# andreadiiorio/SpMV_openMP_CUDA

Measured on AMD Instinct MI355X. Metric: spmv_gflops, higher is better.
Workload: dtype f64

## Files before the change

### include/spmvHip.h

```cpp
#ifndef SPMV_HIP_H
#define SPMV_HIP_H

#include "spmv_types.h"

#ifdef __cplusplus
extern "C" {
#endif

int spmvHipInit(int dev, size_t sizeofSpmat, size_t sizeofConfig);
int spmvHipFinalize(void);
int spmvHipDeviceCount(void);
int spmvHipSetStream(void* stream);
int spmvHipSetSync(int sync);
double spmvHipLastKernelSeconds(void);
int spmvHipLastLaunch(spmvDim3* grid, spmvDim3* block);
int spmvHipDeviceSynchronize(void);

int spmvHipVecAlloc(double** dVec, size_t n);
int spmvHipVecFree(double* dVec);
int spmvHipVecUp(double* dVec, const double* hVec, size_t n);
int spmvHipVecDown(double* hVec, const double* dVec, size_t n);
int spmvHipVecFill(double* dVec, size_t n, uint64_t pattern);

int spmvHipMalloc(void** dPtr, size_t bytes);
// ... 349 lines not shown
    int      taper, ntStore;
    unsigned chunk;
    double   buildMs;
    size_t   bytes;
    double   allocMs;
    size_t   tempBytes;
    int      deterministic;
} spmvTilesInfo;
int spmvHipTilesInfo(spmat* dMat, spmvTilesInfo* info);
int spmvHipTilesBinRow(spmat* dMat, unsigned bin, ulong* firstRow);
int hipSpMVTilesExpand(spmat* dMat, double* dX);
int hipSpMVTilesReduce(spmat* dMat, unsigned binBegin, unsigned binEnd, double* dY, int nExtra, double* const* dExtra);
int hipSpMVTilesReducePush(spmat* dMat, double* dY, int nExtra, double* const* dExtra);
int spmvHipTilesPushJoin(void);
int spmvHipTilesPushFailed(spmat* dMat);

int spmvHipSynthFillCSR(ulong M, ulong N, ulong rowOffset, const void* dIRP, int irpBytes,
                        uint32_t* dJA, double* dAS, uint64_t seedStruct, uint64_t seedVal,
                        ulong band);

#ifdef __cplusplus
}
#endif
#endif
```

### spmv_openmp_cuda_amd/api.py

```python
import contextlib
import ctypes as C
import math
import os

import numpy as np

from .ctypes_defs import CONFIG, POISON_NAN, SPMAT_TAG_ELL_TRANSPOSED, spmat, spmvDim3

_HERE = os.path.dirname(os.path.abspath(__file__))
LIB_PATH = os.environ.get("SPMV_LIB") or os.path.join(_HERE, "lib", "libspmvhip.so")
HOSTLIB_PATH = os.path.join(_HERE, "lib", "libspmvhost.so")


class SpmvHipError(RuntimeError):
    pass


def _load(path):
    if not os.path.exists(path):
        raise SpmvHipError(
            f"{path} is missing: build it with `make lib host` (or __graft_entry__.build()). "
            "This package has no CPU fallback.")
    return C.CDLL(path, mode=C.RTLD_GLOBAL)

# ... 50 lines not shown
    "spmvHipDropCache": ([], _i),
    "spmvHipEventCreate": ([C.POINTER(_vp)], _i), "spmvHipEventDestroy": ([_vp], _i),
    "spmvHipEventRecord": ([_vp], _i), "spmvHipEventElapsedMs": ([_vp, _vp, C.POINTER(C.c_float)], _i),
    "spmvHipPartitionRows": ([_vp, C.c_ulong, _i, _vp], _i),
    "spmvHipRowBlockCSR": ([C.POINTER(spmat), C.c_ulong, C.c_ulong], C.POINTER(spmat)),
    "spmvHipSynthFillCSR": ([C.c_ulong, C.c_ulong, C.c_ulong, _vp, _i, _vp, _vp, _u64, _u64, C.c_ulong], _i),
    "spmvHipCompactRows": ([_vp, _vp, _vp, _i, C.c_ulong], _i),
    "spmvHipWindowCreate": ([_sz, C.POINTER(_vp), _vp], _i), "spmvHipWindowFree": ([_vp], _i),
    "spmvHipWindowOpen": ([_vp, _i, C.POINTER(_vp)], _i), "spmvHipWindowClose": ([_vp], _i),
    "spmvHipPeerPush": ([_vp, _sz, _sz, _i, _vp], _i), "spmvHipPeerPushJoin": ([], _i),
    "spmvHipTilesShape": ([C.POINTER(spmat), C.POINTER(C.c_uint), C.POINTER(C.c_uint)], _i),
    "hipSpMVTilesExpand": ([C.POINTER(spmat), _vp], _i),
    "hipSpMVTilesReduce": ([C.POINTER(spmat), C.c_uint, C.c_uint, _vp, _i, _vp], _i),
    "hipSpMVTilesReducePush": ([C.POINTER(spmat), _vp, _i, _vp], _i), "spmvHipTilesPushFailed": ([C.POINTER(spmat)], _i),
    "spmvHipTilesPushJoin": ([], _i),
    "spmvHipBuildTilesOpt": ([C.POINTER(spmat), _vp], _i), "spmvHipTilesInfo": ([C.POINTER(spmat), _vp], _i),
    "spmvHipTilesBinRow": ([C.POINTER(spmat), C.c_uint, C.POINTER(C.c_ulong)], _i),
    "spmvHipUpdateValues": ([C.POINTER(spmat), _vp, _i], _i), "spmvHipValuesChanged": ([C.POINTER(spmat)], _i),
    "spmvHipLastUpdateInfo": ([C.POINTER(spmat), _vp], _i), "spmvHipShardUpdateValues": ([_vp, _vp], _i),
    "hipSpMMRowsCSR": ([C.POINTER(spmat), C.c_uint, _vp, _sz, _i, _vp, _sz, _i], _i),
    "spmvHipCsrTranspose": ([C.POINTER(spmat), C.POINTER(spmat)], _i),
    "spmvHipTransposeRefresh": ([C.POINTER(spmat), C.POINTER(spmat)], _i),
    "spmvHipTriAnalyse": ([C.POINTER(spmat), _i], _i),
    "hipSpTRSVCSR": ([C.POINTER(spmat), _i, _i, _vp, _vp], _i),
    "spmvHipTriInfo": ([C.POINTER(spmat), _i, _vp], _i),
    "hipSpTRSMCSR": ([C.POINTER(spmat), _i, _i, C.c_uint, _vp, _sz, _i, _vp, _sz, _i], _i),
    "hipSpILU0CSR": ([C.POINTER(spmat)], _i),
    "spmvHipIlu0Info": ([C.POINTER(spmat), _vp], _i),
    "spmvHipDot": ([_sz, _vp, _vp, _vp], _i),
    "hipSpCGCSR": ([C.POINTER(spmat), C.POINTER(spmat), _vp, _vp, _vp, _vp], _i),
# ... 1122 lines not shown
    fn = SPMV_LAUNCHERS[launcher]
    _check(fn(C.byref(dmat.handle), dx.ptr, cfg if cfg is not None else CONFIG(), dy.ptr), launcher)


def build_tiles(dmat: DeviceMatrix, rowsPerBin=0, taper=False, ntStore=-1, chunk=0, deterministic=False):
    o = spmvTilesOpts(int(rowsPerBin), 1 if taper else 0, int(ntStore), int(chunk), 1 if deterministic else 0)
    _check(lib.spmvHipBuildTilesOpt(C.byref(dmat.handle), C.byref(o)), "spmvHipBuildTilesOpt")


def tiles_info(dmat: DeviceMatrix) -> spmvTilesInfo:
    info = spmvTilesInfo()
    _check(lib.spmvHipTilesInfo(C.byref(dmat.handle), C.byref(info)), "spmvHipTilesInfo")
    return info


def build_stripes(dmat: DeviceMatrix, rowsPerBin=0, grid=0, spread=-1, wide=-1, deterministic=False):
    o = spmvStripesOpts(int(rowsPerBin), int(grid), int(spread), int(wide), int(deterministic))
    _check(lib.spmvHipBuildStripesOpt(C.byref(dmat.handle), C.byref(o)), "spmvHipBuildStripesOpt")


def stripes_info(dmat: DeviceMatrix) -> spmvStripesInfo:
    info = spmvStripesInfo()
    _check(lib.spmvHipStripesInfo(C.byref(dmat.handle), C.byref(info)), "spmvHipStripesInfo")
    return info


def dot(u, v):
    with _Operands("dot", u, host_calls=False) as ops:
        n = ops.vector("u", u)
        ops.vector("v", v, n)
# ... 43 lines not shown
```

### spmv_openmp_cuda_amd/csrc/hip/device_mat.hpp

```cpp
#pragma once
#include <hip/hip_runtime.h>
#include <atomic>
#include <cstdint>
#include <cstdio>
#include <type_traits>
#include <vector>

#include "spmvHip.h"

namespace spmvhip {

constexpr int      WAVE            = 64;
constexpr int      WG_THREADS      = 256;
constexpr int      STREAM_NNZ      = 2048;
constexpr uint64_t IRP32_LIMIT     = (1ull << 32) - 65536;

enum class Kind : int { CSR = 0, ELL_ROWMAJOR = 1, ELL_COLMAJOR = 2 };
enum class Origin : int { UPLOADED, ADOPTED, ELL_OF_CSR, TRANSPOSE, PERMUTATION, PRODUCT, HIERARCHY, SUM, FILTER, ASSEMBLED };

struct TileFormat;
struct SellFormat;
struct StripeFormat;
struct SpgemmPlan;
struct AddPlan;
// ... 81 lines not shown
int  enqueueStripes(const StripeFormat* f, const double* x, double* y, hipStream_t stream, int mode, dim3* grid = nullptr, dim3* block = nullptr);
size_t stripesBytes(const DevMat* d);
void stripesInfo(const StripeFormat* f, spmvStripesInfo* out);

int  buildTiles(DevMat* d, const spmvTilesOpts* opts = nullptr);
void tilesInfo(const TileFormat* t, spmvTilesInfo* out);
void freeTiles(TileFormat* t);
void peerFinalize();
void freeTilesWorkspace();
int  enqueueTiles(const DevMat* d, const TileFormat* t, const double* x, double* y, hipStream_t stream);
int  enqueueTilesExpand(const DevMat* d, const TileFormat* t, const double* x, hipStream_t stream);
int  enqueueTilesReduce(const DevMat* d, const TileFormat* t, uint32_t binBegin, uint32_t binEnd, double* y, int nExtra, double* const* extra,
                        hipStream_t stream);
int  enqueueTilesReducePush(const DevMat* d, TileFormat* t, double* y, int nExtra, double* const* extra, hipStream_t stream, hipStream_t side,
                            hipEvent_t evFork, hipEvent_t evJoin);
int  tilesPushFailed(const TileFormat* t);
void tilesShape(const TileFormat* t, uint32_t* bins, uint32_t* rowsPerBin);
uint32_t tilesPhase2Threads(const TileFormat* t);
uint64_t tilesBinRow(const DevMat* d, const TileFormat* t, uint32_t bin);
hipStream_t libraryStream();
size_t tilesBytes(const DevMat* d);

int  tilesRefreshValues(DevMat* d, TileFormat* t, hipStream_t stream, double* mapMs, int* mapsBuilt);
int  stripesRefreshValues(DevMat* d, StripeFormat* f, hipStream_t stream, double* mapMs, int* mapsBuilt);
bool stripesHasValues(const StripeFormat* f);
spmvStripesOpts stripesOptions(const StripeFormat* f);
void stripesSetUnit(StripeFormat* f, bool unit, double value);
int  sellRefreshValues(DevMat* d, hipStream_t stream);
int  transposeCsr(const DevMat* a, DevMat* t, hipStream_t stream);
void enqueueSortedBounds(uint64_t nnz, uint64_t N, const uint32_t* keys, uint32_t* ptr, hipStream_t stream);
// ... 121 lines not shown
```

### spmv_openmp_cuda_amd/csrc/hip/launch.hip

```cpp
#include <hip/hip_runtime.h>

#include "lib.hpp"

using namespace spmvhip;

namespace {

unsigned blockThreads(const CONFIG& cfg, unsigned dflt, unsigned maxThreads) {
    unsigned t = cfg.blockSize.x * std::max(1u, cfg.blockSize.y) * std::max(1u, cfg.blockSize.z);
    if (cfg.blockSize.x == 0) return dflt;
    if (t % WAVE != 0 || t > maxThreads) {
        ERR("CONFIG.blockSize %ux%ux%u is not a multiple of the 64-lane wavefront (or exceeds %u): using %u",
            cfg.blockSize.x, cfg.blockSize.y, cfg.blockSize.z, maxThreads, dflt);
        return dflt;
    }
    return t;
}

template <bool SEQ>
void launchStream2(hipStream_t stream, DevMat* d, double* x, double* y) {
    withIrp(d, [&](auto irp) {
        const auto kernel = d->unit ? csr_stream2_kernel<IrpT<decltype(irp)>, SEQ, true> : csr_stream2_kernel<IrpT<decltype(irp)>, SEQ, false>;
        hipLaunchKernelGGL(kernel, grid2d(d->nBlk2, WG_THREADS), dim3(WG_THREADS), 0, stream,
                           d->nBlk2, d->nLong2, d->blkInfo, d->blkBase, irp, d->JA, d->AS, d->unitValue, x, y);
// ... 293 lines not shown
}

int hipSpMVTilesReduce(spmat* dMat, unsigned binBegin, unsigned binEnd, double* dY, int nExtra, double* const* dExtra) {
    const Ctx cx = libraryCtx();
    const auto [d, t] = tilesReady(dMat, "hipSpMVTilesReduce");
    if (!t) return EXIT_FAILURE;
    uint32_t b = 0, r = 0;
    tilesShape(t, &b, &r);
    if (binBegin > binEnd || binEnd > b || nExtra < 0 || nExtra > SPMV_MAX_PEERS || (nExtra && !dExtra) || !dY) {
        ERR("hipSpMVTilesReduce: bins [%u,%u) of %u, %d extra destinations: invalid", binBegin, binEnd, b, nExtra);
        return EXIT_FAILURE;
    }
    Launch L(cx, dim3(binEnd - binBegin ? binEnd - binBegin : 1), dim3(1024));
    if (enqueueTilesReduce(d, t, binBegin, binEnd, dY, nExtra, dExtra, cx.stream)) { ERR("hipSpMVTilesReduce: launch failed"); return EXIT_FAILURE; }
    return L.finish("hipSpMVTilesReduce");
}

int hipSpMVTilesReducePush(spmat* dMat, double* dY, int nExtra, double* const* dExtra) {
    const Ctx cx = libraryCtx();
    const auto [d, t] = tilesReady(dMat, "hipSpMVTilesReducePush");
    if (!t) return EXIT_FAILURE;
    if (nExtra < 1 || nExtra > SPMV_MAX_PEERS || !dExtra || !dY) { ERR("hipSpMVTilesReducePush: %d destinations: invalid", nExtra); return EXIT_FAILURE; }
    if (!g_pushSide) {
        int lo = 0, hi = 0;
        HIP_TRY(hipDeviceGetStreamPriorityRange(&lo, &hi));
        HIP_TRY(hipStreamCreateWithPriority(&g_pushSide, hipStreamNonBlocking, hi));
        HIP_TRY(hipEventCreateWithFlags(&g_pushFork, hipEventDisableTiming));
        HIP_TRY(hipEventCreateWithFlags(&g_pushJoin, hipEventDisableTiming));
    }
    uint32_t b = 0, r = 0;
// ... 37 lines not shown
```

### spmv_openmp_cuda_amd/csrc/hip/tiles.hip

```cpp
#include <hip/hip_runtime.h>
#include <cstring>
#include <cmath>
#include <chrono>
#include <algorithm>
#include <vector>

#include "spmvHip.h"
#include "kernels.hpp"
#include "device_prims.hpp"

namespace spmvhip {

constexpr uint32_t PB_CBITS   = 14;
constexpr uint32_t PB_C       = 1u << PB_CBITS;
static_assert(PB_C % 1024 == 0 && PB_C * 8 <= 160 * 1024 && PB_C <= 65536, "slice width");
constexpr uint32_t PB_R_MAX   = 20000;
constexpr uint32_t PB_CUS_DEFAULT = 256;
constexpr uint32_t PB_CHUNK   = 1u << 17;
constexpr int      PB_THREADS = 1024;
constexpr uint32_t PD_WAVES   = 4;
constexpr int      PD_THREADS = PD_WAVES * 64;
constexpr size_t   PB_RESIDENT_BYTES = 288ull << 20;

struct BinMap {
// ... 12 lines not shown
struct TileFormat {
    uint32_t S = 0, B = 0, R = 0;
    BinMap    bins;
    uint64_t nnz = 0;
    void*     slab = nullptr;
    double*   val = nullptr;
    uint16_t* lcol = nullptr;
    uint16_t* lrow = nullptr;
    bool      det = false;
    uint32_t* pidx = nullptr;
    size_t    tempBytes = 0;
    uint2*    tl = nullptr;
    uint32_t  nList = 0;
    uint32_t* binPos = nullptr;
    uint32_t* waveTile = nullptr;
    uint3*    work = nullptr;
    uint32_t  nWork = 0;
    uint32_t* runs = nullptr;
    uint32_t  grid1 = 0;
    bool      ntStore = true;
    uint32_t* ready = nullptr;
    uint32_t* pushFail = nullptr;
    uint32_t  epoch = 0;
    uint32_t  cus = PB_CUS_DEFAULT;
    size_t    bytes = 0;
    spmvTilesOpts opts{0, 0, -1, 0, 0};
    uint32_t apiBins() const { return det ? (B + PD_WAVES - 1) / PD_WAVES : B; }
    uint32_t apiRows() const { return det ? PD_WAVES * bins.c : R; }
    BinMap   apiMap() const { if (!det) return bins; BinMap m; m.c = PD_WAVES * bins.c; return m; }
    uint32_t  chunk = 0;
    double    buildMs = 0;
    double    allocMs = 0;
    uint32_t* vmap = nullptr;
};

struct TileDst { double* p[SPMV_MAX_PEERS]; uint32_t n; };
struct TileSignal { uint32_t* ready; uint32_t epoch; };

namespace {

__device__ __forceinline__ uint64_t lin_block() { return (uint64_t)blockIdx.y * gridDim.x + blockIdx.x; }

struct PbPay { uint32_t vlo, vhi, row; };
static_assert(sizeof(PbPay) == 12 && alignof(PbPay) == 4, "payload layout");
__host__ __device__ __forceinline__ PbPay pb_pack(double v, uint32_t row) {
    uint64_t b;
    memcpy(&b, &v, 8);
    return PbPay{(uint32_t)b, (uint32_t)(b >> 32), row};
}
__host__ __device__ __forceinline__ double pb_value(const PbPay& e) {
    const uint64_t b = ((uint64_t)e.vhi << 32) | e.vlo;
    double v;
    memcpy(&v, &b, 8);
    return v;
}

// ... 58 lines not shown
    uint32_t S, uint32_t B, BinMap bm, const uint32_t* __restrict__ tileStart, const uint32_t* __restrict__ bmStart,
    double* __restrict__ val, uint16_t* __restrict__ lcol, uint16_t* __restrict__ lrow, uint32_t* __restrict__ pidx) {
    const uint64_t p = lin_block() * 256 + threadIdx.x;
    if (p >= nnz) return;
    const PbPay e = spay[p];
    const uint32_t key = skeys[p];
    const uint32_t bin = bm.binOf(e.row), slice = key >> PB_CBITS;
    val[p] = pb_value(e);
    lcol[p] = (uint16_t)(key & (PB_C - 1));
    const uint32_t within = (uint32_t)p - tileStart[(uint64_t)slice * B + bin];
    const uint32_t at = bmStart[(uint64_t)bin * S + slice] + within;
    lrow[at] = (uint16_t)(e.row - bm.row0(bin));
    if (pidx) pidx[at] = (uint32_t)p;
}

__global__ __launch_bounds__(256) void pb_fill_kernel(uint32_t* p, uint64_t n, uint32_t v) {
    const uint64_t i = lin_block() * 256 + threadIdx.x;
    if (i < n) p[i] = v;
}

__global__ __launch_bounds__(256) void pb_invert_kernel(uint64_t n, const uint32_t* __restrict__ perm, uint32_t* __restrict__ inv) {
    const uint64_t p = lin_block() * 256 + threadIdx.x;
    if (p < n) inv[perm[p]] = (uint32_t)p;
}

typedef double   dbl2 __attribute__((ext_vector_type(2)));
typedef uint16_t ush2 __attribute__((ext_vector_type(2)));

constexpr int      P1_DEPTH = 8;
constexpr uint32_t P1_STEP  = 2 * PB_THREADS;
// ... 39 lines not shown

template <uint32_t I0, uint32_t I1>
__device__ __forceinline__ void p1_load_x(double (&xv)[I1 - I0], uint32_t slice, const double* __restrict__ x, uint64_t N) {
    const double* xb = x + (uint64_t)slice * PB_C;
    const uint32_t nIn = (uint32_t)min(N - (uint64_t)slice * PB_C, (uint64_t)PB_C);
#pragma unroll
    for (uint32_t i = I0; i < I1; ++i)
        xv[i - I0] = xb[min(threadIdx.x + i * PB_THREADS, nIn - 1)];
}
template <uint32_t I0, uint32_t I1>
__device__ __forceinline__ void p1_fill_x(double* xs, const double (&xv)[I1 - I0]) {
#pragma unroll
    for (uint32_t i = I0; i < I1; ++i) xs[threadIdx.x + i * PB_THREADS] = xv[i - I0];
}

template <bool NT, bool UNIT>
__global__ __launch_bounds__(PB_THREADS) void pb_expand_kernel(
    const uint32_t* __restrict__ runs, const uint3* __restrict__ work, const double* __restrict__ val,
    const uint16_t* __restrict__ lcol, const double* __restrict__ x, uint64_t N, double* __restrict__ prod, double unitValue) {
    extern __shared__ double xs[];
    constexpr uint32_t BATCH = P1_DEPTH * P1_STEP;
    uint32_t item = runs[blockIdx.x];
    const uint32_t itemEnd = runs[blockIdx.x + 1];
    if (item >= itemEnd) return;
    const uint32_t lane2 = 2 * threadIdx.x;

    uint3 w = work[item];
    P1Range r = p1_range(w);
    P1Regs cur, nxt;
    double xv[P1_XPRE];
    p1_load_x<0, P1_XPRE>(xv, w.x, x, N);
    p1_load<UNIT>(cur, r.vb + lane2, r.ve, val, lcol, unitValue);
    bool restage = true;

    for (;;) {
        if (restage) {
            __syncthreads();
            double xr[P1_XALL - P1_XPRE];
// ... 14 lines not shown
        uint32_t pb = r.vb;
        do {
            last = pb + 2 * BATCH >= r.ve;
            const uint32_t p = pb + lane2;
            p1_load<UNIT>(nxt, p + BATCH, r.ve, val, lcol, unitValue);
            p1_store<NT>(cur, p, r.ve, xs, prod);
            if (last && restage) p1_load_x<0, P1_XPRE>(xv, wn.x, x, N);
            const bool hand = last && more;
            p1_load<UNIT>(cur, hand ? rn.vb + lane2 : p + 2 * BATCH, hand ? rn.ve : r.ve, val, lcol, unitValue);
            p1_store<NT>(nxt, p + BATCH, r.ve, xs, prod);
            pb += 2 * BATCH;
        } while (!last);
        if (!more) break;
        w = wn; r = rn; ++item;
    }
}

constexpr int      P2_DEPTH = 8;
constexpr uint32_t P2_WAVES = PB_THREADS / 64;
constexpr uint16_t P2_NONE  = 0xFFFF;
constexpr uint32_t P2_RUNS_FLAG = 0x80000000u;
constexpr uint32_t TL_PAD   = 4;

__host__ __device__ __forceinline__ uint32_t p2_sub(uint32_t len) { return ((len + P2_WAVES - 1) / P2_WAVES + 63u) & ~63u; }

struct P2Regs { double pv[P2_DEPTH]; uint16_t rv[P2_DEPTH]; };
struct P2Cursor { uint32_t k, delta; uint2 n1, n2; };

__device__ __forceinline__ void p2_fetch(P2Regs& r, P2Cursor& c, uint32_t vbase, uint32_t we, uint32_t lane,
                                         const uint2* __restrict__ tl, const double* __restrict__ prod,
// ... 55 lines not shown
            for (uint32_t k = threadIdx.x; k < R; k += THREADS)
                if (r0 + k < M) dst[r0 + k] = yb[k];
        }
    }
    if (MODE == 2) {
        asm volatile("s_waitcnt vmcnt(0)" ::: "memory");
        __syncthreads();
        if (threadIdx.x == 0) {
            __builtin_amdgcn_fence(__ATOMIC_RELEASE, "agent");
            asm volatile("s_waitcnt vmcnt(0)" ::: "memory");
            __hip_atomic_store(sig.ready + bin, sig.epoch, __ATOMIC_RELAXED, __HIP_MEMORY_SCOPE_AGENT);
        }
    }
}

template <int MODE>
__global__ __launch_bounds__(PB_THREADS) void pb_reduce_kernel(
    BinMap bm, uint32_t binBegin, uint32_t binEnd, uint64_t M, const uint32_t* __restrict__ binPos, const uint32_t* __restrict__ waveTile,
    const uint2* __restrict__ tl, const double* __restrict__ prod, const uint16_t* __restrict__ lrow,
    double* __restrict__ y, TileDst extra, TileSignal sig) {
    extern __shared__ double yb[];
    const uint64_t bin = binBegin + lin_block();
    if (bin >= binEnd) return;
    const uint32_t wave = (uint32_t)__builtin_amdgcn_readfirstlane((int)(threadIdx.x / 64)), lane = threadIdx.x % 64;
    const uint32_t v0 = binPos[bin], v1 = binPos[bin + 1];
    const uint32_t sub = p2_sub(v1 - v0);
    const uint32_t wb = v0 + wave * sub, we = min(v1, wb + sub);
    P2Cursor c;
    P2Regs a, b;
    bool runs = false;
    const bool busy = wave * sub < v1 - v0;
    if (busy) {
        const uint32_t wt = waveTile[bin * P2_WAVES + wave];
        runs = (wt & P2_RUNS_FLAG) != 0;
        c.k = wt & ~P2_RUNS_FLAG;
        c.delta = tl[c.k].y;
        c.n1 = tl[c.k + 1];
        c.n2 = tl[c.k + 2];
// ... 15 lines not shown
                    if (b.rv[u] != P2_NONE) atomicAdd(&yb[b.rv[u]], b.pv[u]);
            }
        } else {
            for (uint32_t v = wb; v < we; v += 2 * P2_DEPTH * 64) {
                p2_fetch(b, c, v + P2_DEPTH * 64, we, lane, tl, prod, lrow);
#pragma unroll
                for (int u = 0; u < P2_DEPTH; ++u) p2_add_runs(yb, a.rv[u], a.pv[u], lane);
                p2_fetch(a, c, v + 2 * P2_DEPTH * 64, we, lane, tl, prod, lrow);
#pragma unroll
                for (int u = 0; u < P2_DEPTH; ++u) p2_add_runs(yb, b.rv[u], b.pv[u], lane);
            }
        }
    }
    __syncthreads();
    p2_finish<MODE, PB_THREADS>(yb, R, bm.row0((uint32_t)bin), M, y, extra, sig, (uint32_t)bin);
}

constexpr int PD_DEPTH = 8;
struct PdStream { uint32_t idx[PD_DEPTH]; uint16_t row[PD_DEPTH]; uint32_t first; };
struct PdGather { double p[PD_DEPTH]; };

__device__ __forceinline__ void pd_stream(PdStream& s, uint32_t vb, uint32_t we, uint32_t lane, const uint32_t* __restrict__ pidx,
                                          const uint16_t* __restrict__ lrow) {
    s.first = vb;
#pragma unroll
    for (int u = 0; u < PD_DEPTH; ++u) {
        const uint32_t v = vb + 64u * u + lane, vc = min(v, we - 1u);
        s.idx[u] = __builtin_nontemporal_load(pidx + vc);
        const uint16_t r = __builtin_nontemporal_load(lrow + vc);
        s.row[u] = v < we ? r : P2_NONE;
// ... 1 lines not shown
}
__device__ __forceinline__ void pd_gather(PdGather& g, const PdStream& s, const double* __restrict__ prod) {
#pragma unroll
    for (int u = 0; u < PD_DEPTH; ++u) g.p[u] = prod[s.idx[u]];
}
__device__ __forceinline__ void pd_add(double* yw, const PdStream& s, const PdGather& g) {
#pragma unroll
    for (int u = 0; u < PD_DEPTH; ++u)
        if (s.row[u] != P2_NONE) atomicAdd(&yw[s.row[u]], g.p[u]);
}

template <int MODE>
__global__ __launch_bounds__(PD_THREADS) void pb_reduce_det_kernel(
    BinMap bm, uint32_t nSub, uint32_t binBegin, uint32_t binEnd, uint64_t M, const uint32_t* __restrict__ binPos,
    const uint32_t* __restrict__ pidx, const double* __restrict__ prod, const uint16_t* __restrict__ lrow,
    double* __restrict__ y, TileDst extra, TileSignal sig) {
    extern __shared__ double yb[];
    const uint64_t bin = binBegin + lin_block();
    if (bin >= binEnd) return;
    const uint32_t wave = (uint32_t)__builtin_amdgcn_readfirstlane((int)(threadIdx.x / 64)), lane = threadIdx.x % 64;
    const uint32_t sb = (uint32_t)bin * PD_WAVES + wave;
    const uint32_t Rs = bm.c;
    double* yw = yb + wave * Rs;
    uint32_t wb = 0, we = 0;
    if (sb < nSub) { wb = binPos[sb]; we = binPos[sb + 1]; }
    const bool busy = we > wb;
    constexpr uint32_t BATCH = PD_DEPTH * 64;
    PdStream a, b, c, d;
    PdGather g0, g1;
    if (busy) {
        pd_stream(a, wb, we, lane, pidx, lrow);
        pd_stream(b, wb + BATCH, we, lane, pidx, lrow);
        pd_stream(c, wb + 2 * BATCH, we, lane, pidx, lrow);
    }
// ... 182 lines not shown
            if (g_prod[d].lastUse) (void)hipEventDestroy(g_prod[d].lastUse);
            g_prod[d] = ProdWorkspace{};
        }
    (void)hipSetDevice(keep);
}

uint64_t tilesBinRow(const DevMat* d, const TileFormat* t, uint32_t bin) {
    if (!t) return 0;
    return bin >= t->apiBins() ? d->M : std::min<uint64_t>(d->M, t->apiMap().row0(bin));
}

void freeTiles(TileFormat* t) {
    if (!t) return;
    (void)devFree(t->slab); (void)devFree(t->tl); (void)devFree(t->pidx); (void)devFree(t->vmap);
    (void)devFree(t->binPos); (void)devFree(t->waveTile); (void)devFree(t->work); (void)devFree(t->runs); (void)devFree(t->ready);
    delete t;
}

static int buildFailed(const char* what) { (void)hipGetLastError(); fprintf(stderr, "libspmvhip: tiles: %s failed\n", what); return EXIT_FAILURE; }

static int checkTilesBuild(const DevMat* d, const spmvTilesOpts& o) {
    if (d->kind != Kind::CSR) return EXIT_FAILURE;
    if (o.deterministic && o.taper) { fprintf(stderr, "libspmvhip: tiles: the deterministic form has no tapered bins\n"); return EXIT_FAILURE; }
    if (o.rowsPerBin != 0 && (o.rowsPerBin < 64 || o.rowsPerBin > PB_R_MAX)) {
        fprintf(stderr, "libspmvhip: tiles: rowsPerBin = %u is not 0 (automatic) or 64..%u\n", o.rowsPerBin, PB_R_MAX);
        return EXIT_FAILURE;
    }
    if (o.chunk != 0 && (o.chunk < 4096 || o.chunk > (1u << 24))) {
        fprintf(stderr, "libspmvhip: tiles: chunk = %u is not 0 (automatic) or 4096..2^24\n", o.chunk);
        return EXIT_FAILURE;
// ... 118 lines not shown
        TempBuf dupCount;
        if (dupCount.alloc((size_t)t->B * P2_WAVES * 4)) return buildFailed("run-count workspace");
        HIP_TRY(hipMemsetAsync(dupCount.p, 0, (size_t)t->B * P2_WAVES * 4, nullptr));
        hipLaunchKernelGGL(pb_dupcount_kernel, grid2d((nnz + 255) / 256, 256), dim3(256), 0, nullptr, t->B, nnz, t->binPos, t->lrow,
                           dupCount.as<uint32_t>());
        hipLaunchKernelGGL(pb_wavetile_kernel, grid2d(((uint64_t)t->B * P2_WAVES + 255) / 256, 256), dim3(256), 0, nullptr, t->B,
                           t->binPos, binTile.as<uint32_t>(), t->tl, dupCount.as<uint32_t>(), t->waveTile);
        HIP_TRY(hipGetLastError());
        HIP_TRY(hipDeviceSynchronize());
    }
    HIP_TRY(hipGetLastError());
    HIP_TRY(hipDeviceSynchronize());
    return EXIT_SUCCESS;
}

static uint32_t phase1Chunk(const std::vector<uint32_t>& sliceStart, uint64_t nnz, uint32_t PB_CUS) {
    uint32_t chunk = PB_CHUNK;
    uint64_t nonEmpty = 0;
    for (size_t s = 0; s + 1 < sliceStart.size(); ++s) nonEmpty += sliceStart[s + 1] > sliceStart[s];
    const double avgLen = nonEmpty ? (double)nnz / (double)nonEmpty : 1.0;
    double bestCost = 1e300;
    const uint32_t pLo = (uint32_t)std::max(1.0, std::ceil(avgLen / 100000.0));
    const uint32_t pHi = (uint32_t)std::max((double)pLo, std::ceil(avgLen / 50000.0));
    for (uint32_t p = pLo; p <= std::min<uint32_t>(pHi, 1024); ++p) {
        const double rounds = (double)nonEmpty * p / PB_CUS;
        const double waste = (std::ceil(rounds) - rounds) / rounds;
        const double cost = 0.35 * waste + 0.1 * p * (PB_C * 8.0) / (avgLen * 18.0);
        if (cost < bestCost) { bestCost = cost; chunk = (uint32_t)std::min(16777216.0, std::ceil(avgLen / p * 1.02) + 64); }
    }
    return chunk;
// ... 28 lines not shown
            if (c > b) { plan.work.push_back(make_uint3(it.x, b, c)); b = c; }
            plan.runs[g] = (uint32_t)plan.work.size();
        }
        plan.work.push_back(make_uint3(it.x, b, it.z));
    }
    for (; g <= grid; ++g) plan.runs[g] = (uint32_t)plan.work.size();
    return plan;
}

static int setTilesKernelAttributes() {
    const struct { const void* kernel; int ldsBytes; } attrs[] = {
        {(const void*)pb_expand_kernel<true, false>, PB_C * 8}, {(const void*)pb_expand_kernel<false, false>, PB_C * 8},
        {(const void*)pb_expand_kernel<true, true>, PB_C * 8},  {(const void*)pb_expand_kernel<false, true>, PB_C * 8},
        {(const void*)pb_reduce_kernel<0>, PB_R_MAX * 8},       {(const void*)pb_reduce_kernel<1>, PB_R_MAX * 8},
        {(const void*)pb_reduce_kernel<2>, PB_R_MAX * 8},       {(const void*)pb_reduce_det_kernel<0>, PB_R_MAX * 8},
        {(const void*)pb_reduce_det_kernel<1>, PB_R_MAX * 8},   {(const void*)pb_reduce_det_kernel<2>, PB_R_MAX * 8}};
    for (const auto& a : attrs) HIP_TRY(hipFuncSetAttribute(a.kernel, hipFuncAttributeMaxDynamicSharedMemorySize, a.ldsBytes));
    return EXIT_SUCCESS;
}

int buildTiles(DevMat* d, const spmvTilesOpts* opts) {
    const spmvTilesOpts o = opts ? *opts : spmvTilesOpts{0, 0, -1, 0, 0};
    TileFormat*& slot = d->tiles[o.deterministic != 0];
    if (slot && !opts) return EXIT_SUCCESS;
    if (checkTilesBuild(d, o)) return EXIT_FAILURE;
    if (slot) { freeTiles(slot); slot = nullptr; }
    const uint64_t nnz = d->NZ;
    TileFormat* t = new TileFormat;
    struct Guard { TileFormat*& t; ~Guard() { if (t) freeTiles(t); } } guard{t};
    {
        int dev = 0, cus = 0;
// ... 2 lines not shown
    }
    hipEvent_t ev0 = nullptr, ev1 = nullptr;
    HIP_TRY(hipEventCreate(&ev0));
    HIP_TRY(hipEventCreate(&ev1));
    struct EvGuard { hipEvent_t a, b; ~EvGuard() { (void)hipEventDestroy(a); (void)hipEventDestroy(b); } } evGuard{ev0, ev1};
    HIP_TRY(hipEventRecord(ev0, nullptr));
    const TileGeometry g = planTileBins(d->M, t->cus, o);
    t->opts = o;
    t->S = (uint32_t)((d->N + PB_C - 1) / PB_C);
    t->bins = g.bins; t->R = g.R; t->B = g.B;
    t->det = o.deterministic != 0;
    t->nnz = nnz;
    if ((uint64_t)t->S * t->B >= (1ull << 32) - 2) { fprintf(stderr, "libspmvhip: tiles: too many tiles\n"); return EXIT_FAILURE; }

    TileBuildTemps tmp;
    if (sortIntoSlices(d, t, tmp) || placeTiles(t, tmp)) return EXIT_FAILURE;

    std::vector<uint32_t> sliceStart(t->S + 1);
    HIP_TRY(hipMemcpy2D(sliceStart.data(), 4, tmp.tileStart.as<uint32_t>(), (size_t)t->B * 4, 4, t->S + 1, hipMemcpyDeviceToHost));
    t->chunk = o.chunk ? o.chunk : phase1Chunk(sliceStart, nnz, t->cus);
    const Phase1Plan plan = planPhase1Work(sliceStart, t->chunk, t->cus);
    t->nWork = (uint32_t)plan.work.size();
    t->grid1 = plan.runs.empty() ? 0 : (uint32_t)plan.runs.size() - 1;
    HIP_TRY(devMalloc(&t->work, std::max<size_t>(plan.work.size(), 1) * sizeof(uint3)));
    HIP_TRY(hipMemcpy(t->work, plan.work.data(), plan.work.size() * sizeof(uint3), hipMemcpyHostToDevice));
    HIP_TRY(devMalloc(&t->runs, std::max<size_t>(plan.runs.size(), 1) * sizeof(uint32_t)));
    HIP_TRY(hipMemcpy(t->runs, plan.runs.data(), plan.runs.size() * sizeof(uint32_t), hipMemcpyHostToDevice));
    HIP_TRY(hipDeviceSynchronize());

    if (setTilesKernelAttributes()) return EXIT_FAILURE;
    t->ntStore = o.ntStore >= 0 ? o.ntStore != 0 : nnz * 8 > PB_RESIDENT_BYTES;
// ... 46 lines not shown
void tilesInfo(const TileFormat* t, spmvTilesInfo* out) {
    memset(out, 0, sizeof *out);
    if (!t) return;
    out->nBins = t->apiBins(); out->rowsPerBin = t->apiRows(); out->nSlices = t->S; out->taper = t->bins.n1 != 0; out->ntStore = t->ntStore;
    out->chunk = t->chunk; out->buildMs = t->buildMs; out->bytes = t->bytes; out->allocMs = t->allocMs;
    out->tempBytes = t->tempBytes; out->deterministic = t->det ? 1 : 0;
}

uint32_t tilesPhase2Threads(const TileFormat* t) { return t && t->det ? (uint32_t)PD_THREADS : (uint32_t)PB_THREADS; }

void tilesShape(const TileFormat* t, uint32_t* bins, uint32_t* rowsPerBin) {
    *bins = t ? t->apiBins() : 0;
    *rowsPerBin = t ? t->apiRows() : 0;
}

int enqueueTilesExpand(const DevMat* d, const TileFormat* t, const double* x, hipStream_t stream) {
    if (!t) return EXIT_FAILURE;
    double* prod = prodWorkspace(t->nnz, true);
    if (!prod || prodHandover(stream)) return EXIT_FAILURE;
    if (t->nWork) {
#define PB_EXPAND(NT, UNIT) hipLaunchKernelGGL((pb_expand_kernel<NT, UNIT>), dim3(t->grid1), dim3(PB_THREADS), PB_C * 8, stream, t->runs, t->work, \
                                              t->val, t->lcol, x, d->N, prod, d->unitValue)
        if (d->unit) { if (t->ntStore) PB_EXPAND(true, true); else PB_EXPAND(false, true); }
        else         { if (t->ntStore) PB_EXPAND(true, false); else PB_EXPAND(false, false); }
#undef PB_EXPAND
    }
    return hipGetLastError() == hipSuccess ? EXIT_SUCCESS : EXIT_FAILURE;
}

int enqueueTilesReduce(const DevMat* d, const TileFormat* t, uint32_t binBegin, uint32_t binEnd, double* y, int nExtra, double* const* extra,
                       hipStream_t stream) {
    if (!t || binBegin > binEnd || binEnd > t->apiBins() || nExtra < 0 || nExtra > SPMV_MAX_PEERS) return EXIT_FAILURE;
    if (binBegin == binEnd) return EXIT_SUCCESS;
    const dim3 grid = grid2d((uint64_t)((binEnd - binBegin + 7) / 8) * 8, PB_THREADS);
    const double* prod = prodWorkspace(t->nnz, false);
    if (!prod || prodHandover(stream)) return EXIT_FAILURE;
    TileDst dst{};
    dst.n = (uint32_t)nExtra;
    for (int i = 0; i < nExtra; ++i) dst.p[i] = extra[i];
    const TileSignal none{nullptr, 0};
    if (t->det) {
        const size_t lds = (size_t)8 * t->apiRows();
        if (nExtra)
            hipLaunchKernelGGL(pb_reduce_det_kernel<1>, grid, dim3(PD_THREADS), lds, stream, t->bins, t->B, binBegin, binEnd, d->M, t->binPos,
                               t->pidx, prod, t->lrow, y, dst, none);
        else
            hipLaunchKernelGGL(pb_reduce_det_kernel<0>, grid, dim3(PD_THREADS), lds, stream, t->bins, t->B, binBegin, binEnd, d->M, t->binPos,
                               t->pidx, prod, t->lrow, y, dst, none);
        const bool launched = hipGetLastError() == hipSuccess;
        prodMark(stream);
        return launched ? EXIT_SUCCESS : EXIT_FAILURE;
    }
    if (nExtra)
        hipLaunchKernelGGL(pb_reduce_kernel<1>, grid, dim3(PB_THREADS), (size_t)8 * t->R, stream,
                           t->bins, binBegin, binEnd, d->M, t->binPos, t->waveTile, t->tl, prod, t->lrow, y, dst, none);
    else
        hipLaunchKernelGGL(pb_reduce_kernel<0>, grid, dim3(PB_THREADS), (size_t)8 * t->R, stream,
                           t->bins, binBegin, binEnd, d->M, t->binPos, t->waveTile, t->tl, prod, t->lrow, y, dst, none);
    const bool launched = hipGetLastError() == hipSuccess;
    prodMark(stream);
    return launched ? EXIT_SUCCESS : EXIT_FAILURE;
}

int enqueueTilesReducePush(const DevMat* d, TileFormat* t, double* y, int nExtra, double* const* extra, hipStream_t stream, hipStream_t side,
                           hipEvent_t evFork, hipEvent_t evJoin) {
    if (!t || nExtra < 1 || nExtra > SPMV_MAX_PEERS) return EXIT_FAILURE;
    const double* prod = prodWorkspace(t->nnz, true);
    if (!prod || prodHandover(stream)) return EXIT_FAILURE;
    const uint32_t nb = t->apiBins();
    if (!t->ready) {
        if (!hipOk(devMalloc(&t->ready, ((size_t)nb + 1) * 4), "hipMalloc of the bins' ready flags")) return EXIT_FAILURE;
        if (hipMemset(t->ready, 0, ((size_t)nb + 1) * 4) != hipSuccess) return EXIT_FAILURE;
        t->pushFail = t->ready + nb;
    }
    const uint32_t epoch = ++t->epoch ? t->epoch : ++t->epoch;
    TileDst dst{};
    dst.n = (uint32_t)nExtra;
    for (int i = 0; i < nExtra; ++i) dst.p[i] = extra[i];
    const TileSignal sig{t->ready, epoch};
    if (hipEventRecord(evFork, stream) != hipSuccess || hipStreamWaitEvent(side, evFork, 0) != hipSuccess) return EXIT_FAILURE;
    hipLaunchKernelGGL(pb_push_kernel, dim3(std::min<uint32_t>(PUSH_WGS, nb)), dim3(PUSH_THREADS), 0, side, t->apiMap(), nb, d->M, t->ready,
                       epoch, y, dst, t->pushFail);
    if (t->det)
        hipLaunchKernelGGL(pb_reduce_det_kernel<2>, grid2d((uint64_t)((nb + 7) / 8) * 8, PB_THREADS), dim3(PD_THREADS), (size_t)8 * t->apiRows(), stream,
                           t->bins, t->B, 0u, nb, d->M, t->binPos, t->pidx, prod, t->lrow, y, TileDst{}, sig);
    else
        hipLaunchKernelGGL(pb_reduce_kernel<2>, grid2d((uint64_t)((t->B + 7) / 8) * 8, PB_THREADS), dim3(PB_THREADS), (size_t)8 * t->R, stream,
                           t->bins, 0u, t->B, d->M, t->binPos, t->waveTile, t->tl, prod, t->lrow, y, TileDst{}, sig);
    const bool launched = hipGetLastError() == hipSuccess;
    prodMark(stream);
    if (hipEventRecord(evJoin, side) != hipSuccess) return EXIT_FAILURE;
    return launched ? EXIT_SUCCESS : EXIT_FAILURE;
}

int tilesPushFailed(const TileFormat* t) {
    if (!t || !t->pushFail) return 0;
    uint32_t f = 0;
    if (hipMemcpy(&f, t->pushFail, 4, hipMemcpyDeviceToHost) != hipSuccess) return 1;
    return f != 0;
}

int enqueueTiles(const DevMat* d, const TileFormat* t, const double* x, double* y, hipStream_t stream) {
    if (!t) return EXIT_FAILURE;
    if (enqueueTilesExpand(d, t, x, stream)) return EXIT_FAILURE;
    return enqueueTilesReduce(d, t, 0, t->apiBins(), y, 0, nullptr, stream);
}

}
```

Baseline: 402.3.

## Schedule reduce bins heaviest-first via sorted bin order and add stamp probes

At build time the bins are sorted by descending nonzero count, and the reduce kernels index bins through this order when they cover the whole range. The longest bins therefore start first, which is meant to cut tail imbalance in the reduce phase. The change also adds wall-clock stamp instrumentation entry points for per-workgroup timing. The cost is one extra indirection load per workgroup and a sort step during build.

After: 394.4. -2.0%, worse.

```diff
diff --git a/include/spmvHip.h b/include/spmvHip.h
--- a/include/spmvHip.h
+++ b/include/spmvHip.h
@@ -387,6 +387,8 @@
 int hipSpMVTilesReducePush(spmat* dMat, double* dY, int nExtra, double* const* dExtra);
 int spmvHipTilesPushJoin(void);
 int spmvHipTilesPushFailed(spmat* dMat);
+int spmvHipTilesFinishSpread(spmat* dMat, double* dX, double* dY, double out[6]);
+int spmvHipTilesFinishStamps(spmat* dMat, int phase, unsigned cap, double* entryUs, double* exitUs, unsigned* count);
 
 int spmvHipSynthFillCSR(ulong M, ulong N, ulong rowOffset, const void* dIRP, int irpBytes,
                         uint32_t* dJA, double* dAS, uint64_t seedStruct, uint64_t seedVal,
diff --git a/spmv_openmp_cuda_amd/api.py b/spmv_openmp_cuda_amd/api.py
--- a/spmv_openmp_cuda_amd/api.py
+++ b/spmv_openmp_cuda_amd/api.py
@@ -88,6 +88,8 @@
     "hipSpMVTilesReduce": ([C.POINTER(spmat), C.c_uint, C.c_uint, _vp, _i, _vp], _i),
     "hipSpMVTilesReducePush": ([C.POINTER(spmat), _vp, _i, _vp], _i), "spmvHipTilesPushFailed": ([C.POINTER(spmat)], _i),
     "spmvHipTilesPushJoin": ([], _i),
+    "spmvHipTilesFinishSpread": ([C.POINTER(spmat), _vp, _vp, C.POINTER(C.c_double)], _i),
+    "spmvHipTilesFinishStamps": ([C.POINTER(spmat), _i, C.c_uint, _vp, _vp, C.POINTER(C.c_uint)], _i),
     "spmvHipBuildTilesOpt": ([C.POINTER(spmat), _vp], _i), "spmvHipTilesInfo": ([C.POINTER(spmat), _vp], _i),
     "spmvHipTilesBinRow": ([C.POINTER(spmat), C.c_uint, C.POINTER(C.c_ulong)], _i),
     "spmvHipUpdateValues": ([C.POINTER(spmat), _vp, _i], _i), "spmvHipValuesChanged": ([C.POINTER(spmat)], _i),
@@ -1240,6 +1242,20 @@
     return info
 
 
+def tiles_finish_spread(dmat: DeviceMatrix, dx: DeviceVector, dy: DeviceVector):
+    out = (C.c_double * 6)()
+    _check(lib.spmvHipTilesFinishSpread(C.byref(dmat.handle), dx.ptr, dy.ptr, out), "spmvHipTilesFinishSpread")
+    stamps = []
+    for phase in (0, 1):
+        n = C.c_uint(0)
+        _check(lib.spmvHipTilesFinishStamps(C.byref(dmat.handle), phase, 0, None, None, C.byref(n)), "spmvHipTilesFinishStamps")
+        entry, exit_ = np.zeros(n.value), np.zeros(n.value)
+        _check(lib.spmvHipTilesFinishStamps(C.byref(dmat.handle), phase, n.value, entry.ctypes.data, exit_.ctypes.data, C.byref(n)),
+               "spmvHipTilesFinishStamps")
+        stamps.append((entry, exit_))
+    return np.array(out[:]), stamps
+
+
 def build_stripes(dmat: DeviceMatrix, rowsPerBin=0, grid=0, spread=-1, wide=-1, deterministic=False):
     o = spmvStripesOpts(int(rowsPerBin), int(grid), int(spread), int(wide), int(deterministic))
     _check(lib.spmvHipBuildStripesOpt(C.byref(dmat.handle), C.byref(o)), "spmvHipBuildStripesOpt")
diff --git a/spmv_openmp_cuda_amd/csrc/hip/device_mat.hpp b/spmv_openmp_cuda_amd/csrc/hip/device_mat.hpp
--- a/spmv_openmp_cuda_amd/csrc/hip/device_mat.hpp
+++ b/spmv_openmp_cuda_amd/csrc/hip/device_mat.hpp
@@ -119,6 +119,8 @@
                         hipStream_t stream);
 int  enqueueTilesReducePush(const DevMat* d, TileFormat* t, double* y, int nExtra, double* const* extra, hipStream_t stream, hipStream_t side,
                             hipEvent_t evFork, hipEvent_t evJoin);
+int  tilesFinishSpread(const DevMat* d, TileFormat* t, const double* x, double* y, hipStream_t stream, double out[6]);
+int  tilesFinishStamps(const TileFormat* t, int phase, uint32_t cap, double* entryUs, double* exitUs, uint32_t* count);
 int  tilesPushFailed(const TileFormat* t);
 void tilesShape(const TileFormat* t, uint32_t* bins, uint32_t* rowsPerBin);
 uint32_t tilesPhase2Threads(const TileFormat* t);
diff --git a/spmv_openmp_cuda_amd/csrc/hip/launch.hip b/spmv_openmp_cuda_amd/csrc/hip/launch.hip
--- a/spmv_openmp_cuda_amd/csrc/hip/launch.hip
+++ b/spmv_openmp_cuda_amd/csrc/hip/launch.hip
@@ -331,6 +331,24 @@
     Launch L(cx, dim3(binEnd - binBegin ? binEnd - binBegin : 1), dim3(1024));
     if (enqueueTilesReduce(d, t, binBegin, binEnd, dY, nExtra, dExtra, cx.stream)) { ERR("hipSpMVTilesReduce: launch failed"); return EXIT_FAILURE; }
     return L.finish("hipSpMVTilesReduce");
+}
+
+int spmvHipTilesFinishSpread(spmat* dMat, double* dX, double* dY, double out[6]) {
+    const Ctx cx = libraryCtx();
+    DevMat* d = csrOf(dMat, dX, dY, "spmvHipTilesFinishSpread");
+    if (!d || !out || !nonEmptyCsr(d, "spmvHipTilesFinishSpread")) return EXIT_FAILURE;
+    TileFormat* t = ensureTiles(d, false);
+    if (!t) return EXIT_FAILURE;
+    if (tilesFinishSpread(d, t, dX, dY, cx.stream, out)) { ERR("spmvHipTilesFinishSpread: the stamped launches failed"); return EXIT_FAILURE; }
+    return EXIT_SUCCESS;
+}
+
+int spmvHipTilesFinishStamps(spmat* dMat, int phase, unsigned cap, double* entryUs, double* exitUs, unsigned* count) {
+    DevMat* d = descOf(dMat, "spmvHipTilesFinishStamps");
+    uint32_t n = 0;
+    if (!d || !count || tilesFinishStamps(d->tiles[0], phase, cap, entryUs, exitUs, &n)) return EXIT_FAILURE;
+    *count = n;
+    return EXIT_SUCCESS;
 }
 
 int hipSpMVTilesReducePush(spmat* dMat, double* dY, int nExtra, double* const* dExtra) {
diff --git a/spmv_openmp_cuda_amd/csrc/hip/tiles.hip b/spmv_openmp_cuda_amd/csrc/hip/tiles.hip
--- a/spmv_openmp_cuda_amd/csrc/hip/tiles.hip
+++ b/spmv_openmp_cuda_amd/csrc/hip/tiles.hip
@@ -50,6 +50,7 @@
     uint32_t  nList = 0;
     uint32_t* binPos = nullptr;
     uint32_t* waveTile = nullptr;
+    uint32_t* binOrder = nullptr;
     uint3*    work = nullptr;
     uint32_t  nWork = 0;
     uint32_t* runs = nullptr;
@@ -68,6 +69,8 @@
     double    buildMs = 0;
     double    allocMs = 0;
     uint32_t* vmap = nullptr;
+    unsigned long long* stamps = nullptr;
+    std::vector<double> stampUs[2][2];
 };
 
 struct TileDst { double* p[SPMV_MAX_PEERS]; uint32_t n; };
@@ -76,6 +79,12 @@
 namespace {
 
 __device__ __forceinline__ uint64_t lin_block() { return (uint64_t)blockIdx.y * gridDim.x + blockIdx.x; }
+
+__device__ __forceinline__ void p_stamp_exit(unsigned long long* slot) {
+    asm volatile("s_waitcnt vmcnt(0)" ::: "memory");
+    __syncthreads();
+    if (threadIdx.x == 0) *slot = wall_clock64();
+}
 
 struct PbPay { uint32_t vlo, vhi, row; };
 static_assert(sizeof(PbPay) == 12 && alignof(PbPay) == 4, "payload layout");
@@ -164,6 +173,14 @@
     if (pidx) pidx[at] = (uint32_t)p;
 }
 
+__global__ __launch_bounds__(256) void pb_binkeys_kernel(uint32_t nb, uint32_t per, uint32_t B, const uint32_t* __restrict__ binPos,
+                                                         uint32_t* __restrict__ keys) {
+    const uint64_t i = lin_block() * 256 + threadIdx.x;
+    if (i >= nb) return;
+    const uint64_t lo = i * per, hi = min((i + 1) * per, (uint64_t)B);
+    keys[i] = ~(binPos[hi] - binPos[lo]);
+}
+
 __global__ __launch_bounds__(256) void pb_fill_kernel(uint32_t* p, uint64_t n, uint32_t v) {
     const uint64_t i = lin_block() * 256 + threadIdx.x;
     if (i < n) p[i] = v;
@@ -233,14 +250,16 @@
     for (uint32_t i = I0; i < I1; ++i) xs[threadIdx.x + i * PB_THREADS] = xv[i - I0];
 }
 
-template <bool NT, bool UNIT>
+template <bool NT, bool UNIT, bool STAMP = false>
 __global__ __launch_bounds__(PB_THREADS) void pb_expand_kernel(
     const uint32_t* __restrict__ runs, const uint3* __restrict__ work, const double* __restrict__ val,
-    const uint16_t* __restrict__ lcol, const double* __restrict__ x, uint64_t N, double* __restrict__ prod, double unitValue) {
+    const uint16_t* __restrict__ lcol, const double* __restrict__ x, uint64_t N, double* __restrict__ prod, double unitValue,
+    unsigned long long* __restrict__ stamps) {
     extern __shared__ double xs[];
     constexpr uint32_t BATCH = P1_DEPTH * P1_STEP;
     uint32_t item = runs[blockIdx.x];
     const uint32_t itemEnd = runs[blockIdx.x + 1];
+    if (STAMP && threadIdx.x == 0) stamps[2 * blockIdx.x] = stamps[2 * blockIdx.x + 1] = wall_clock64();
     if (item >= itemEnd) return;
     const uint32_t lane2 = 2 * threadIdx.x;
 
@@ -285,6 +304,7 @@
         if (!more) break;
         w = wn; r = rn; ++item;
     }
+    if (STAMP) p_stamp_exit(stamps + 2 * blockIdx.x + 1);
 }
 
 constexpr int      P2_DEPTH = 8;
@@ -370,14 +390,16 @@
     }
 }
 
-template <int MODE>
+template <int MODE, bool STAMP = false>
 __global__ __launch_bounds__(PB_THREADS) void pb_reduce_kernel(
     BinMap bm, uint32_t binBegin, uint32_t binEnd, uint64_t M, const uint32_t* __restrict__ binPos, const uint32_t* __restrict__ waveTile,
     const uint2* __restrict__ tl, const double* __restrict__ prod, const uint16_t* __restrict__ lrow,
-    double* __restrict__ y, TileDst extra, TileSignal sig) {
+    double* __restrict__ y, TileDst extra, TileSignal sig, unsigned long long* __restrict__ stamps, const uint32_t* __restrict__ order) {
     extern __shared__ double yb[];
-    const uint64_t bin = binBegin + lin_block();
-    if (bin >= binEnd) return;
+    const uint64_t turn = binBegin + lin_block();
+    if (turn >= binEnd) return;
+    const uint64_t bin = order ? order[turn] : turn;
+    if (STAMP && threadIdx.x == 0) stamps[2 * lin_block()] = wall_clock64();
     const uint32_t wave = (uint32_t)__builtin_amdgcn_readfirstlane((int)(threadIdx.x / 64)), lane = threadIdx.x % 64;
     const uint32_t v0 = binPos[bin], v1 = binPos[bin + 1];
     const uint32_t sub = p2_sub(v1 - v0);
@@ -423,6 +445,7 @@
     }
     __syncthreads();
     p2_finish<MODE, PB_THREADS>(yb, R, bm.row0((uint32_t)bin), M, y, extra, sig, (uint32_t)bin);
+    if (STAMP) p_stamp_exit(stamps + 2 * lin_block() + 1);
 }
 
 constexpr int PD_DEPTH = 8;
@@ -454,10 +477,11 @@
 __global__ __launch_bounds__(PD_THREADS) void pb_reduce_det_kernel(
     BinMap bm, uint32_t nSub, uint32_t binBegin, uint32_t binEnd, uint64_t M, const uint32_t* __restrict__ binPos,
     const uint32_t* __restrict__ pidx, const double* __restrict__ prod, const uint16_t* __restrict__ lrow,
-    double* __restrict__ y, TileDst extra, TileSignal sig) {
+    double* __restrict__ y, TileDst extra, TileSignal sig, const uint32_t* __restrict__ order) {
     extern __shared__ double yb[];
-    const uint64_t bin = binBegin + lin_block();
-    if (bin >= binEnd) return;
+    const uint64_t turn = binBegin + lin_block();
+    if (turn >= binEnd) return;
+    const uint64_t bin = order ? order[turn] : turn;
     const uint32_t wave = (uint32_t)__builtin_amdgcn_readfirstlane((int)(threadIdx.x / 64)), lane = threadIdx.x % 64;
     const uint32_t sb = (uint32_t)bin * PD_WAVES + wave;
     const uint32_t Rs = bm.c;
@@ -670,6 +694,7 @@
     if (!t) return;
     (void)devFree(t->slab); (void)devFree(t->tl); (void)devFree(t->pidx); (void)devFree(t->vmap);
     (void)devFree(t->binPos); (void)devFree(t->waveTile); (void)devFree(t->work); (void)devFree(t->runs); (void)devFree(t->ready);
+    (void)devFree(t->stamps); (void)devFree(t->binOrder);
     delete t;
 }
 
@@ -818,6 +843,24 @@
     return EXIT_SUCCESS;
 }
 
+static int orderBins(TileFormat* t) {
+    const uint32_t nb = t->apiBins(), per = t->det ? PD_WAVES : 1;
+    TempBuf keys, keysOut, idx, sortTmp;
+    if (keys.alloc((size_t)nb * 4) || keysOut.alloc((size_t)nb * 4) || idx.alloc((size_t)nb * 4) || devMalloc(&t->binOrder, (size_t)nb * 4)) {
+        t->binOrder = nullptr;
+        return buildFailed("bin-order allocation");
+    }
+    t->bytes += (size_t)nb * 4;
+    hipLaunchKernelGGL(pb_binkeys_kernel, grid2d(((uint64_t)nb + 255) / 256, 256), dim3(256), 0, nullptr, nb, per, t->B, t->binPos, keys.as<uint32_t>());
+    enqueueIota(nb, idx.as<uint32_t>(), nullptr);
+    if (sortPairs(sortTmp, keys.as<uint32_t>(), keysOut.as<uint32_t>(), idx.as<uint32_t>(), t->binOrder, (size_t)nb, 0, 32, nullptr) != hipSuccess ||
+        hipGetLastError() != hipSuccess || hipDeviceSynchronize() != hipSuccess) {
+        (void)hipDeviceSynchronize();
+        return buildFailed("bin-order sort");
+    }
+    return EXIT_SUCCESS;
+}
+
 static uint32_t phase1Chunk(const std::vector<uint32_t>& sliceStart, uint64_t nnz, uint32_t PB_CUS) {
     uint32_t chunk = PB_CHUNK;
     uint64_t nonEmpty = 0;
@@ -876,7 +919,10 @@
         {(const void*)pb_expand_kernel<true, true>, PB_C * 8},  {(const void*)pb_expand_kernel<false, true>, PB_C * 8},
         {(const void*)pb_reduce_kernel<0>, PB_R_MAX * 8},       {(const void*)pb_reduce_kernel<1>, PB_R_MAX * 8},
         {(const void*)pb_reduce_kernel<2>, PB_R_MAX * 8},       {(const void*)pb_reduce_det_kernel<0>, PB_R_MAX * 8},
-        {(const void*)pb_reduce_det_kernel<1>, PB_R_MAX * 8},   {(const void*)pb_reduce_det_kernel<2>, PB_R_MAX * 8}};
+        {(const void*)pb_reduce_det_kernel<1>, PB_R_MAX * 8},   {(const void*)pb_reduce_det_kernel<2>, PB_R_MAX * 8},
+        {(const void*)pb_expand_kernel<true, false, true>, PB_C * 8}, {(const void*)pb_expand_kernel<false, false, true>, PB_C * 8},
+        {(const void*)pb_expand_kernel<true, true, true>, PB_C * 8},  {(const void*)pb_expand_kernel<false, true, true>, PB_C * 8},
+        {(const void*)pb_reduce_kernel<0, true>, PB_R_MAX * 8}};
     for (const auto& a : attrs) HIP_TRY(hipFuncSetAttribute(a.kernel, hipFuncAttributeMaxDynamicSharedMemorySize, a.ldsBytes));
     return EXIT_SUCCESS;
 }
@@ -909,7 +955,7 @@
     if ((uint64_t)t->S * t->B >= (1ull << 32) - 2) { fprintf(stderr, "libspmvhip: tiles: too many tiles\n"); return EXIT_FAILURE; }
 
     TileBuildTemps tmp;
-    if (sortIntoSlices(d, t, tmp) || placeTiles(t, tmp)) return EXIT_FAILURE;
+    if (sortIntoSlices(d, t, tmp) || placeTiles(t, tmp) || orderBins(t)) return EXIT_FAILURE;
 
     std::vector<uint32_t> sliceStart(t->S + 1);
     HIP_TRY(hipMemcpy2D(sliceStart.data(), 4, tmp.tileStart.as<uint32_t>(), (size_t)t->B * 4, 4, t->S + 1, hipMemcpyDeviceToHost));
@@ -986,18 +1032,25 @@
     *rowsPerBin = t ? t->apiRows() : 0;
 }
 
+template <bool STAMP>
+static void launchExpand(const DevMat* d, const TileFormat* t, const double* x, double* prod, hipStream_t stream, unsigned long long* stamps) {
+#define PB_EXPAND(NT, UNIT) hipLaunchKernelGGL((pb_expand_kernel<NT, UNIT, STAMP>), dim3(t->grid1), dim3(PB_THREADS), PB_C * 8, stream, t->runs, t->work, \
+                                              t->val, t->lcol, x, d->N, prod, d->unitValue, stamps)
+    if (d->unit) { if (t->ntStore) PB_EXPAND(true, true); else PB_EXPAND(false, true); }
+    else         { if (t->ntStore) PB_EXPAND(true, false); else PB_EXPAND(false, false); }
+#undef PB_EXPAND
+}
+
 int enqueueTilesExpand(const DevMat* d, const TileFormat* t, const double* x, hipStream_t stream) {
     if (!t) return EXIT_FAILURE;
     double* prod = prodWorkspace(t->nnz, true);
     if (!prod || prodHandover(stream)) return EXIT_FAILURE;
-    if (t->nWork) {
-#define PB_EXPAND(NT, UNIT) hipLaunchKernelGGL((pb_expand_kernel<NT, UNIT>), dim3(t->grid1), dim3(PB_THREADS), PB_C * 8, stream, t->runs, t->work, \
-                                              t->val, t->lcol, x, d->N, prod, d->unitValue)
-        if (d->unit) { if (t->ntStore) PB_EXPAND(true, true); else PB_EXPAND(false, true); }
-        else         { if (t->ntStore) PB_EXPAND(true, false); else PB_EXPAND(false, false); }
-#undef PB_EXPAND
-    }
+    if (t->nWork) launchExpand<false>(d, t, x, prod, stream, nullptr);
     return hipGetLastError() == hipSuccess ? EXIT_SUCCESS : EXIT_FAILURE;
+}
+
+static const uint32_t* wholeRangeOrder(const TileFormat* t, uint32_t binBegin, uint32_t binEnd) {
+    return binBegin == 0 && binEnd == t->apiBins() && t->bins.n1 == 0 ? t->binOrder : nullptr;
 }
 
 int enqueueTilesReduce(const DevMat* d, const TileFormat* t, uint32_t binBegin, uint32_t binEnd, double* y, int nExtra, double* const* extra,
@@ -1011,24 +1064,25 @@
     dst.n = (uint32_t)nExtra;
     for (int i = 0; i < nExtra; ++i) dst.p[i] = extra[i];
     const TileSignal none{nullptr, 0};
+    const uint32_t* const order = wholeRangeOrder(t, binBegin, binEnd);
     if (t->det) {
         const size_t lds = (size_t)8 * t->apiRows();
         if (nExtra)
             hipLaunchKernelGGL(pb_reduce_det_kernel<1>, grid, dim3(PD_THREADS), lds, stream, t->bins, t->B, binBegin, binEnd, d->M, t->binPos,
-                               t->pidx, prod, t->lrow, y, dst, none);
+                               t->pidx, prod, t->lrow, y, dst, none, nullptr);
         else
             hipLaunchKernelGGL(pb_reduce_det_kernel<0>, grid, dim3(PD_THREADS), lds, stream, t->bins, t->B, binBegin, binEnd, d->M, t->binPos,
-                               t->pidx, prod, t->lrow, y, dst, none);
+                               t->pidx, prod, t->lrow, y, dst, none, order);
         const bool launched = hipGetLastError() == hipSuccess;
         prodMark(stream);
         return launched ? EXIT_SUCCESS : EXIT_FAILURE;
     }
     if (nExtra)
         hipLaunchKernelGGL(pb_reduce_kernel<1>, grid, dim3(PB_THREADS), (size_t)8 * t->R, stream,
-                           t->bins, binBegin, binEnd, d->M, t->binPos, t->waveTile, t->tl, prod, t->lrow, y, dst, none);
+                           t->bins, binBegin, binEnd, d->M, t->binPos, t->waveTile, t->tl, prod, t->lrow, y, dst, none, nullptr, nullptr);
     else
         hipLaunchKernelGGL(pb_reduce_kernel<0>, grid, dim3(PB_THREADS), (size_t)8 * t->R, stream,
-                           t->bins, binBegin, binEnd, d->M, t->binPos, t->waveTile, t->tl, prod, t->lrow, y, dst, none);
+                           t->bins, binBegin, binEnd, d->M, t->binPos, t->waveTile, t->tl, prod, t->lrow, y, dst, none, nullptr, order);
     const bool launched = hipGetLastError() == hipSuccess;
     prodMark(stream);
     return launched ? EXIT_SUCCESS : EXIT_FAILURE;
@@ -1055,10 +1109,10 @@
                        epoch, y, dst, t->pushFail);
     if (t->det)
         hipLaunchKernelGGL(pb_reduce_det_kernel<2>, grid2d((uint64_t)((nb + 7) / 8) * 8, PB_THREADS), dim3(PD_THREADS), (size_t)8 * t->apiRows(), stream,
-                           t->bins, t->B, 0u, nb, d->M, t->binPos, t->pidx, prod, t->lrow, y, TileDst{}, sig);
+                           t->bins, t->B, 0u, nb, d->M, t->binPos, t->pidx, prod, t->lrow, y, TileDst{}, sig, nullptr);
     else
         hipLaunchKernelGGL(pb_reduce_kernel<2>, grid2d((uint64_t)((t->B + 7) / 8) * 8, PB_THREADS), dim3(PB_THREADS), (size_t)8 * t->R, stream,
-                           t->bins, 0u, t->B, d->M, t->binPos, t->waveTile, t->tl, prod, t->lrow, y, TileDst{}, sig);
+                           t->bins, 0u, t->B, d->M, t->binPos, t->waveTile, t->tl, prod, t->lrow, y, TileDst{}, sig, nullptr, nullptr);
     const bool launched = hipGetLastError() == hipSuccess;
     prodMark(stream);
     if (hipEventRecord(evJoin, side) != hipSuccess) return EXIT_FAILURE;
@@ -1078,4 +1132,55 @@
     return enqueueTilesReduce(d, t, 0, t->apiBins(), y, 0, nullptr, stream);
 }
 
-}
+int tilesFinishSpread(const DevMat* d, TileFormat* t, const double* x, double* y, hipStream_t stream, double out[6]) {
+    if (!t || t->det) return EXIT_FAILURE;
+    const uint32_t n[2] = {t->nWork ? t->grid1 : 0u, t->B};
+    const size_t words = 2 * ((size_t)n[0] + n[1]);
+    if (!t->stamps && devMalloc(&t->stamps, words * sizeof(unsigned long long)) != hipSuccess) { t->stamps = nullptr; return buildFailed("stamp buffer allocation"); }
+    double* prod = prodWorkspace(t->nnz, true);
+    if (!prod || prodHandover(stream)) return EXIT_FAILURE;
+    HIP_TRY(hipMemsetAsync(t->stamps, 0, words * sizeof(unsigned long long), stream));
+    unsigned long long* const s2 = t->stamps + 2 * (size_t)n[0];
+    if (n[0]) launchExpand<true>(d, t, x, prod, stream, t->stamps);
+    hipLaunchKernelGGL((pb_reduce_kernel<0, true>), grid2d((uint64_t)((t->B + 7) / 8) * 8, PB_THREADS), dim3(PB_THREADS), (size_t)8 * t->R, stream,
+                       t->bins, 0u, t->B, d->M, t->binPos, t->waveTile, t->tl, prod, t->lrow, y, TileDst{}, TileSignal{nullptr, 0}, s2, wholeRangeOrder(t, 0, t->B));
+    const bool launched = hipGetLastError() == hipSuccess;
+    prodMark(stream);
+    if (!launched) return EXIT_FAILURE;
+    std::vector<unsigned long long> h(words);
+    HIP_TRY(hipStreamSynchronize(stream));
+    HIP_TRY(hipMemcpy(h.data(), t->stamps, words * sizeof(unsigned long long), hipMemcpyDeviceToHost));
+    int dev = 0, kHz = 0;
+    if (hipGetDevice(&dev) != hipSuccess || hipDeviceGetAttribute(&kHz, hipDeviceAttributeWallClockRate, dev) != hipSuccess || kHz <= 0) {
+        (void)hipGetLastError();
+        kHz = 100000;
+    }
+    const double usPerTick = 1e3 / kHz;
+    const unsigned long long* s = h.data();
+    for (int ph = 0; ph < 2; ++ph, s += 2 * (size_t)n[ph - 1]) {
+        std::vector<double>&in = t->stampUs[ph][0], &ex = t->stampUs[ph][1];
+        in.assign(n[ph], 0.0); ex.assign(n[ph], 0.0);
+        out[3 * ph] = out[3 * ph + 1] = out[3 * ph + 2] = 0.0;
+        if (!n[ph]) continue;
+        unsigned long long t0 = s[0];
+        for (uint32_t g = 0; g < n[ph]; ++g) t0 = std::min(t0, s[2 * g]);
+        for (uint32_t g = 0; g < n[ph]; ++g) { in[g] = (double)(s[2 * g] - t0) * usPerTick; ex[g] = (double)(s[2 * g + 1] - t0) * usPerTick; }
+        std::vector<double> sorted(ex);
+        std::sort(sorted.begin(), sorted.end());
+        out[3 * ph] = sorted.front(); out[3 * ph + 1] = sorted[sorted.size() / 2]; out[3 * ph + 2] = sorted.back();
+    }
+    return EXIT_SUCCESS;
+}
+
+int tilesFinishStamps(const TileFormat* t, int phase, uint32_t cap, double* entryUs, double* exitUs, uint32_t* count) {
+    if (!t || phase < 0 || phase > 1 || !count) return EXIT_FAILURE;
+    const std::vector<double>&in = t->stampUs[phase][0], &ex = t->stampUs[phase][1];
+    *count = (uint32_t)in.size();
+    for (uint32_t g = 0; g < std::min<size_t>(cap, in.size()); ++g) {
+        if (entryUs) entryUs[g] = in[g];
+        if (exitUs) exitUs[g] = ex[g];
+    }
+    return EXIT_SUCCESS;
+}
+
+}
```
